# Jutho/Strided.jl

Hardware: AMD Instinct MI355X
Metric: GB/s effective HBM for @strided permutedims!+broadcast, 32^4 fp64 (higher is better)
Workload: dtype f64

## Files before the change

### strided.jl_amd/csrc/smr_api.cpp

```cpp
#include <algorithm>
#include <cstdio>
#include <cstring>
#include <atomic>
#include <list>
#include <memory>
#include <mutex>
#include <string>
#include <unordered_map>
#include <vector>

#include "smr_dispatch.h"
#include "smr_group.h"

namespace smr {

static thread_local std::string g_last_error;

int set_error(int code, const std::string& msg) {
    g_last_error = msg;
    return code;
}
int hip_error(hipError_t e, const char* what) {
    g_last_error = std::string(what) + ": " + hipGetErrorString(e);
    return e == hipErrorOutOfMemory ? SMR_ENOMEM : (e == hipErrorNoDevice ? SMR_ENODEVICE : SMR_EHIP);
// ... 316 lines not shown
        const uint32_t align = (uint32_t)((uintptr_t)p->ops[k].base & 255u);
        int32_t acls = k;
        const char* ak = (const char*)p->ops[k].base + p->ops[k].offset * (int64_t)dtype_size(p->ops[k].dtype);
        for (int j = 0; j < k; ++j)
            if ((const char*)p->ops[j].base + p->ops[j].offset * (int64_t)dtype_size(p->ops[j].dtype) == ak) {
                acls = j;
                break;
            }
        put(&acls, sizeof acls);
        put(&cls, sizeof cls);
        put(&align, sizeof align);
        put(&p->ops[k].offset, sizeof(int64_t));
        put(p->ops[k].strides, sizeof(int64_t) * (size_t)p->N);
        put(&p->ops[k].dtype, sizeof(int32_t));
        put(&p->ops[k].conj, sizeof(int32_t));
    }
    put(&p->fprog_len, sizeof(int32_t));
    if (p->fprog && p->fprog_len > 0) put(p->fprog, (size_t)(2 * p->fprog_len));
    put(&p->nconsts, sizeof(int32_t));
    if (p->fconsts && p->nconsts > 0) put(p->fconsts, sizeof(double) * (size_t)(2 * p->nconsts));
    put(&p->redop, sizeof(int32_t));
    put(&p->initop, sizeof(int32_t));
    put(p->initarg, sizeof p->initarg);
    put(&p->stream, sizeof(void*));
    return s;
}

void cache_clear_locked(Cache& c, std::vector<PlanRef>& dropped) {
    for (auto& kv : c.lru) dropped.push_back(std::move(kv.second));
    c.lru.clear();
    c.map.clear();
}

struct OptionField {
    const char* name;
    i64 Options::*field;
};
const OptionField OPTION_FIELDS[] = {
    {"force_family", &Options::force_family},
    {"jit", &Options::jit},
    {"max_lds_bytes", &Options::max_lds_bytes},
    {"tile_log2", &Options::tile_log2},
    {"tile_order", &Options::tile_order},
    {"tile_block", &Options::tile_block},
    {"tile_block_xcd", &Options::tile_block_xcd},
    {"tiled_vec", &Options::tiled_vec},
    {"tiled_uavec", &Options::tiled_uavec},
    {"tiled_edge_first", &Options::tiled_edge_first},
    {"tiled_persist", &Options::tiled_persist},
    {"tiled_persist_wpc", &Options::tiled_persist_wpc},
    {"tiled_persist_min", &Options::tiled_persist_min},
    {"tiled_xpose", &Options::tiled_xpose},
    {"tiled_gorder", &Options::tiled_gorder},
    {"orbit", &Options::orbit},
    {"orbit_lg", &Options::orbit_lg},
    {"orbit_min", &Options::orbit_min},
    {"orbit_few", &Options::orbit_few},
    {"orbit_minrun", &Options::orbit_minrun},
    {"orbit_group", &Options::orbit_group},
    {"orbit_pipe", &Options::orbit_pipe},
    {"orbit_wgs", &Options::orbit_wgs},
    {"orbit_pair", &Options::orbit_pair},
    {"orbit_pack", &Options::orbit_pack},
    {"flat", &Options::flat},
    {"flat_wide", &Options::flat_wide},
    {"flat2", &Options::flat2},
    {"flat2_pair", &Options::flat2_pair},
    {"flat2_bytes", &Options::flat2_bytes},
    {"flat2_lead_bytes", &Options::flat2_lead_bytes},
    {"flat2_long", &Options::flat2_long},
    {"flatb", &Options::flatb},
    {"stream_ua", &Options::stream_ua},
    {"stream_pack_rows", &Options::stream_pack_rows},
    {"nt_store", &Options::nt_store},
    {"nt_stream_min", &Options::nt_stream_min},
    {"reduce_blocks", &Options::reduce_blocks},
    {"reduce_part_wgs", &Options::reduce_part_wgs},
    {"reduce_part_kind", &Options::reduce_part_kind},
    {"reduce_single", &Options::reduce_single},
    {"reduce_row_floor", &Options::reduce_row_floor},
    {"reduce_row_dense", &Options::reduce_row_dense},
    {"reduce_col_txlog", &Options::reduce_col_txlog},
    {"reduce_col_exact", &Options::reduce_col_exact},
    {"reduce_col_narrow", &Options::reduce_col_narrow},
    {"nt_load", &Options::nt_load},
    {"eager_direct", &Options::eager_direct},
    {"eager_self_release", &Options::eager_self_release},
    {"seq_self_release", &Options::seq_self_release},
    {"self_release_max_bytes", &Options::self_release_max_bytes},
    {"self_release_max_total", &Options::self_release_max_total},
    {"allreduce_f64", &Options::allreduce_f64},
};

i64 Options::*option_field(const std::string& n) {
    for (const OptionField& f : OPTION_FIELDS)
        if (n == f.name) return f.field;
    return nullptr;
}

int tile_lg_dim(const std::string& n) {
    return n.size() == 8 && n.rfind("tile_lg", 0) == 0 && n[7] >= '0' && n[7] <= '7' ? n[7] - '0' : -1;
}
}

extern "C" {

// ... 443 lines not shown
```

### strided.jl_amd/csrc/smr_internal.h

```cpp
#pragma once

#ifndef SMR_JIT
#include <hip/hip_runtime.h>

#include <array>
#include <memory>
#include <mutex>
#include <string>
#include <vector>

#include "../../include/strided_hip.h"
#else
#include "strided_hip.h"
#endif

#include <cstdint>

namespace smr {

typedef int64_t i64;
constexpr int MAXN = SMR_MAXN;
constexpr int MAXM = SMR_MAXM;
constexpr int MAXIN = SMR_MAXM - 1;
constexpr int STACK = 8;
constexpr int MAXG = 4;
constexpr int FLATB_MAXP = 512;
constexpr int TILED_NG = 4;

#ifndef SMR_JIT
int set_error(int code, const std::string& msg);
int hip_error(hipError_t e, const char* what);
#endif

inline int dtype_size(int dt) {
    switch (dt) {
        case SMR_F32: return 4;
        case SMR_F64: return 8;
        case SMR_C32: return 8;
        case SMR_C64: return 16;
        case SMR_I8: case SMR_U8: case SMR_BOOL: return 1;
        case SMR_I16: case SMR_U16: return 2;
        case SMR_I32: case SMR_U32: return 4;
        case SMR_I64: case SMR_U64: return 8;
    }
    return 0;
}

struct ProgD {
    int32_t len;
    int32_t nconst;
    uint8_t code[2 * SMR_MAXPROG];
    double consts[2 * SMR_MAXCONST];
};

struct JitConsts {
    double c[2 * SMR_MAXCONST];
};

enum FKind : int {
    FK_PROG = 0,
    FK_IDENT = 1,
    FK_ADD2 = 2,
    FK_ADD3 = 3,
    FK_ADD4 = 4,
    FK_SCALE = 5,
    FK_SYM = 6,
    FK_AXPY = 7,
    FK_AXPBY = 8,
    FK_ABS2 = 9,
    FK_MUL2 = 10,
    FK_EXPR5 = 11,
    FK_COUNT
};

enum Family : int {
    FAM_AUTO = 0,
    FAM_GENERIC = 1,
    FAM_STREAM = 2,
    FAM_TILED = 3,
    FAM_REDUCE_ALL = 4,
// ... 84 lines not shown
};

struct Flat2Plan {
    bool on = false;
    int kt = 1;
    bool shared = false;
    int R[2] = {1, 1}, TP[2] = {1, 1}, p[2] = {-1, -1};
    bool ingroup[2][MAXN] = {{false, false, false, false, false, false, false, false}, {false, false, false, false, false, false, false, false}};
    int32_t roff[2][64];
};

struct FlatBPlan {
    bool on = false;
    int g = 0, P = 0, K = 1;
    uint16_t srcoff[FLATB_MAXP];
};

struct StreamPlan {
    int vec = 1;
    bool vec_ua = false;
};

struct ReducePlan {
    int nparts = 1;
    size_t scratch_bytes = 0;
    int tr = 1;
    int kind = 0;
    int g0log = 0, g1log = 0;
    int txlog = 0;
    int col_tx = 0, col_v = 1;
    int col_y0 = 1, col_y1 = 1;
    int xsplit = 1, qsplit = 1;
};

struct Plan {
    Canon c;
    int family = FAM_GENERIC;
    FlatBPlan flatb;
    TilePlan tile;
    OrbitPlan orbit;
    FlatPlan flat;
    Flat2Plan flat2;
    StreamPlan stream;
    ReducePlan red;
    mutable bool eager_seen = false;
    void* scratch = nullptr;
    size_t counter_off = 0;
    struct FormCache {
        std::vector<unsigned char> args;
        void* tab = nullptr;
    };
    mutable std::shared_ptr<std::mutex> build_mu = std::make_shared<std::mutex>();
    mutable FormCache tiled_cache[4];
    mutable void* tiled_order = nullptr;
    mutable FormCache orbit_cache[2];
    mutable void* orbit_list = nullptr;
    mutable FormCache pair_cache;
    std::array<void**, 9> dev_tables() const {
        return {&tiled_cache[0].tab, &tiled_cache[1].tab, &tiled_cache[2].tab, &tiled_cache[3].tab, &tiled_order,
                &orbit_cache[0].tab, &orbit_cache[1].tab, &orbit_list, &pair_cache.tab};
    }
    struct ArgBlock {
        int launch = 0;
        std::vector<unsigned char> bytes;
        void* dev = nullptr;
        int dev_index = 0;
        unsigned long long epoch = 0;
    };
    mutable std::vector<ArgBlock> eager_args;
    std::string desc;
};

constexpr int RED_COUNTERS = 16384;
struct Options {
    i64 force_family = 0;
    i64 tile_log2 = 0;
    i64 tile_order = 1;
    i64 tile_block = -1;
    i64 tile_block_xcd = -1;
    i64 jit = 1;
    i64 reduce_col_txlog = 5;
    i64 reduce_part_wgs = 1024;
    i64 reduce_row_floor = -1;
    i64 flat_wide = 1;
    i64 flat2 = 1;
    i64 flat2_pair = 1;
    i64 flat2_bytes = 384;
    i64 flat2_lead_bytes = 512;
    i64 reduce_row_dense = 1;
    i64 reduce_col_exact = 1;
    i64 reduce_col_narrow = 1;
    i64 reduce_part_kind = -1;
    i64 reduce_single = 4;
    i64 reduce_blocks = 2048;
    i64 tiled_persist = 1;
    i64 tiled_persist_wpc = 0;
    i64 tiled_persist_min = 32;
    i64 eager_direct = 1;
    i64 flat2_long = 80;
    i64 flatb = 1;
    i64 stream_pack_rows = 1;
    i64 tiled_vec = 1;
    i64 tiled_edge_first = 1;
    i64 tiled_uavec = 1;
    i64 orbit = 1;
    i64 stream_ua = 1;
    i64 tiled_xpose = 1;
    i64 tiled_gorder = -1;
    i64 allreduce_f64 = 0;
    i64 eager_self_release = 1;
    i64 seq_self_release = 1;
    i64 self_release_max_total = (i64)128 << 20;
    i64 self_release_max_bytes = (i64)64 << 20;
    i64 orbit_lg = -1;
    i64 orbit_min = 150;
    i64 orbit_pipe = -1;
    i64 orbit_group = 2;
    i64 stamp_base = 0, stamp_cap = 0, stamp_used = 0;
    i64 flat = 1;
    i64 orbit_minrun = 16;
    i64 orbit_wgs = 0;
    i64 orbit_pair = 1;
    i64 orbit_pack = 1;
    i64 orbit_few = 40;
    i64 nt_store = -1;
    i64 nt_stream_min = 0;
    i64 nt_load = -1;
    i64 max_lds_bytes = 65536;
    i64 tile_lg[MAXN] = {-1, -1, -1, -1, -1, -1, -1, -1};
};
Options& options();

unsigned long long* stamp_next(size_t waves);

int canonicalise(const smr_problem* p, Canon& c);
int make_plan(const smr_problem* p, Plan& plan);
void describe(Plan& plan);

enum RedFold { RED_FOLD_EPILOGUE = 0, RED_FOLD_IN_LAUNCH = 1, RED_FOLD_SECOND_LAUNCH = 2 };
struct RedLaunch {
    int vec = 1;
    int fold = RED_FOLD_EPILOGUE;
    int nparts = 1;
    i64 groups = 0;
    int ctx = 0, cty = 0, cy0 = 0, cy1 = 0;
};
RedLaunch reduce_launch(const Plan& plan, void* const* bases, bool have_scratch);

struct TiledVariant {
    int V = 1;
    bool ua = false;
    int mode = 0;
    bool wide = false;
    int thrlog = 8;
    unsigned pgrid = 0;
};
TiledVariant tiled_variant(const Plan& plan, void* const* bases, int esize, bool mixed);

constexpr int SMR_JIT_UNAVAILABLE = 1000;
struct JitLaunch {
    const char* family;
    const char* tname;
    std::string entry;
    const char* argtype;
    unsigned grid = 1, block = 256;
    size_t lds = 0;
    const void* args = nullptr;
    size_t argsize = 0;
};
int jit_launch(const Canon& c, const JitLaunch& l, hipStream_t s);
int jit_compile_only(const Canon& c, const JitLaunch& l, size_t* code_size);
std::string jit_functor_source(const Canon& c, const char* tname);
bool jit_dry_run();
void jit_set_prepare(bool on);
bool jit_no_launch();
void jit_set_dry_run(bool on);
size_t jit_dry_code_size();
struct JitStats {
    long compiles = 0, hits = 0, failures = 0;
    double compile_ms = 0;
};
JitStats jit_stats();

int fence_for_foreign_work(hipStream_t s);

struct RecLaunch {
    const void* hostfn = nullptr;
    std::string kname;
    std::shared_ptr<void> keep;
    unsigned grid = 0, block = 0, lds = 0;
    int slice_kind = 0;
    unsigned slice_off = 0, slice_row = 0;
    bool self_released = false;
    std::vector<unsigned char> args;
};
std::vector<RecLaunch>* recorder();
struct Plan;
int eager_submit(const Plan& plan, std::vector<RecLaunch>& launches, const std::vector<std::pair<uintptr_t, uintptr_t>>& rd,
                 const std::vector<std::pair<uintptr_t, uintptr_t>>& wr, hipStream_t s);
long comm_stat(int which);
void count_launch();
int eager_fence_all();
void eager_note_hip_work(hipStream_t s);
void eager_forget_stream(hipStream_t s);
void eager_request_sys_acquire(hipStream_t s);
long eager_stat(int which);
bool eager_available(hipStream_t s);
int eager_fence_if_active();
bool eager_recent_writes_fit(uintptr_t dest_lo, uintptr_t dest_hi);
void mark_sliceable(int kind, unsigned off, unsigned row);
void mark_self_released();
void take_slice_mark(RecLaunch& r);
void set_recorder(std::vector<RecLaunch>* r, bool allow_self_release = false, bool eager = false);
bool want_self_release(const Plan& plan);

int upload_table(void** dst, const void* src, size_t bytes, const char* what);
int cu_count();

int launch_generic_map(const Plan& plan, void* const* bases, hipStream_t s);
int launch_stream_map(const Plan& plan, void* const* bases, hipStream_t s);
int launch_tiled_map(const Plan& plan, void* const* bases, hipStream_t s);
int launch_reduce_all(const Plan& plan, void* const* bases, hipStream_t s);
int launch_reduce_part(const Plan& plan, void* const* bases, hipStream_t s);
int launch_orbit_map(const Plan& plan, void* const* bases, hipStream_t s);
int launch_flat_map(const Plan& plan, void* const* bases, hipStream_t s);

#endif

}
```

### strided.jl_amd/csrc/smr_k_tiled.hip

```cpp
#ifndef SMR_JIT
#include <cstdio>
#include <cstdlib>
#include <vector>
#endif

#include "smr_dispatch.h"

#ifndef SMR_CT
#error "compile with -DSMR_CT=0..3 or 7"
#endif
#ifndef SMR_TILED_BITS
#define SMR_TILED_BITS 0
#endif
#ifndef SMR_TILED_NTL
#define SMR_TILED_NTL 0
#endif

namespace smr {

constexpr int MAXT = 5;
constexpr int NG = TILED_NG;
constexpr int EPL = 4;
constexpr int NORD16 = 512;

// ... 1118 lines not shown
    constexpr int T0 = 128, TQ = 32;
    if constexpr (is_jit<F>::value || !tr<T>::arith || sizeof(T) < 8 || (F::NIN >= 0 && F::NIN != 1)) {
        return SMR_EUNSUPPORTED;
    } else {
        if (!options().tiled_xpose) return SMR_EUNSUPPORTED;
        if (c.M != 2 || c.mixed || c.N < 3 || c.N > MAXN || t.nt != 2 || t.tilelog != 12 || t.staged[1] < 0 || !t.ord.empty()) return SMR_EUNSUPPORTED;
        if (t.tdim[0] != 0 || t.tlog[0] != 7 || t.tlog[1] != 5) return SMR_EUNSUPPORTED;
        const int q = t.tdim[1];
        if (c.strides[0][0] != 1 || c.strides[1][q] != 1 || c.dims[0] % T0 || c.dims[q] % TQ) return SMR_EUNSUPPORTED;
        if (tab.conj[0] || tab.conj[1]) return SMR_EUNSUPPORTED;
        if (c.algbytes < ((i64)512 << 20)) return SMR_EUNSUPPORTED;
        const i64 es = (i64)sizeof(T);
        if ((((uintptr_t)tab.base[0]) | ((uintptr_t)tab.base[1])) % 16) return SMR_EUNSUPPORTED;
        for (int d = 0; d < c.N; ++d) {
            if (d != 0 && (c.strides[0][d] * es) % 16) return SMR_EUNSUPPORTED;
            if (d != q && (c.strides[1][d] * es) % 16) return SMR_EUNSUPPORTED;
        }
        XposeArgs a;
        std::memset(&a, 0, sizeof a);
        a.src = (const char*)tab.base[1];
        a.dst = (char*)tab.base[0];
        a.src_row = c.strides[1][0] * es;
        a.dst_row = c.strides[0][q] * es;
        i64 grid = 1;
        int ng = 0;
        for (int i = 0; i < c.N; ++i) {
            const int d = t.gorder[i] >= 0 && t.gorder[i] < c.N ? t.gorder[i] : -1;
            if (d < 0) return SMR_EUNSUPPORTED;
            const i64 tile = d == 0 ? T0 : (d == q ? TQ : 1);
            const i64 n = c.dims[d] / tile;
            if (n <= 1) continue;
            if (n > 0xffffffffLL) return SMR_EUNSUPPORTED;
            a.ext[ng] = (uint32_t)n;
            a.sstep[ng] = c.strides[1][d] * es * tile;
            a.dstep[ng] = c.strides[0][d] * es * tile;
            grid *= n;
            ++ng;
        }
        {
            bool seen[MAXN] = {false};
            for (int i = 0; i < c.N; ++i) {
                if (seen[t.gorder[i]]) return SMR_EUNSUPPORTED;
                seen[t.gorder[i]] = true;
            }
        }
        a.ng = ng;
        if (grid < 1 || grid > 0x7fffffffLL) return SMR_EUNSUPPORTED;
        const size_t lds = (size_t)T0 * (TQ + 2) * sizeof(T);
        auto kern = k_xpose_big<T, F, V, T0, TQ>;
        return launch_native((const void*)kern, lds, "k_xpose_big", [&] { SMR_LAUNCH(kern, dim3((unsigned)grid), dim3(1024), lds, s, a, f); });
    }
}

template <class T, class F, bool MIXED>
static int go(const Plan& plan, void* const* bases, hipStream_t s, F f) {
    const Canon& c = plan.c;
    const TilePlan& t = plan.tile;
    const OpTab tab = make_optab(c, bases);
    if constexpr (!MIXED) {
        const int rc = try_xpose_big<T, F>(plan, s, f, tab);
        if (rc != SMR_EUNSUPPORTED) return rc;
    }
    if (t.tilelog != 10 && t.tilelog != 12) return set_error(SMR_EINVAL, "tiled: the planner must pick 1024- or 4096-element tiles");
    const TiledVariant tv = tiled_variant(plan, bases, (int)sizeof(T), MIXED);
    if (tv.thrlog == 8) return go_tl<T, F, MIXED, 8>(plan, s, f, tab, tv);
    return go_tl<T, F, MIXED, 10>(plan, s, f, tab, tv);
}

template <>
int launch_tiled_map_ct<SMR_CT>(const Plan& plan, void* const* bases, hipStream_t s) {
    typedef ct_type<SMR_CT>::type T;
    const Canon& c = plan.c;
    if (c.bitcopy) return with_bitcopy<SMR_CT>(c, [&](auto f) { return go<typename ident_elem<decltype(f)>::type, decltype(f), false>(plan, bases, s, f); });
    if (c.mixed) return with_prog<T>(c, [&](auto f) { return go<T, decltype(f), true>(plan, bases, s, f); });
    switch (c.fkind) {
        case FK_IDENT: return go<T, FIdent<T>, false>(plan, bases, s, FIdent<T>{});
        case FK_ADD2: return go<T, FAdd2<T>, false>(plan, bases, s, FAdd2<T>{});
        case FK_ADD3: return go<T, FAdd3<T>, false>(plan, bases, s, FAdd3<T>{});
        case FK_ADD4: return go<T, FAdd4<T>, false>(plan, bases, s, FAdd4<T>{});
        case FK_SCALE: return go<T, FScale<T>, false>(plan, bases, s, FScale<T>{hostmk<T>(c.fc[0], c.fc[1])});
        case FK_SYM: return go<T, FSym<T>, false>(plan, bases, s, FSym<T>{hostmk<T>(c.fc[0], c.fc[1])});
        case FK_AXPY: return go<T, FAxpy<T>, false>(plan, bases, s, FAxpy<T>{hostmk<T>(c.fc[0], c.fc[1])});
        case FK_AXPBY:
            return go<T, FAxpby<T>, false>(plan, bases, s, FAxpby<T>{hostmk<T>(c.fc[0], c.fc[1]), hostmk<T>(c.fc[2], c.fc[3])});
        default: break;
    }
    return with_prog<T>(c, [&](auto f) { return go<T, decltype(f), false>(plan, bases, s, f); });
}
#endif

}
```

### strided.jl_amd/csrc/smr_kmeta.cpp

```cpp
#include "smr_kmeta.h"

#include <algorithm>
#include <cstring>
#include <iterator>
#include <vector>

namespace smr {
namespace {

struct Cur {
    const unsigned char* p;
    const unsigned char* end;
    bool bad = false;

    bool need(size_t n) {
        if ((size_t)(end - p) < n) bad = true;
        return !bad;
    }
    uint64_t be(int n) {
        if (!need((size_t)n)) return 0;
        uint64_t v = 0;
        for (int i = 0; i < n; ++i) v = (v << 8) | p[i];
        p += n;
        return v;
// ... 64 lines not shown
                case 0xd9: str((size_t)be(1)); break;
                case 0xda: str((size_t)be(2)); break;
                case 0xdb: str((size_t)be(4)); break;
                case 0xdc: t.kind = ARR; t.i = (int64_t)be(2); break;
                case 0xdd: t.kind = ARR; t.i = (int64_t)be(4); break;
                case 0xde: t.kind = MAP; t.i = (int64_t)be(2); break;
                case 0xdf: t.kind = MAP; t.i = (int64_t)be(4); break;
                default: bad = true; break;
            }
        if (bad) t.kind = BAD;
        return t;
    }
    void skip_value() {
        uint64_t pending = 1;
        while (pending && !bad) {
            const Tok t = next();
            --pending;
            if (t.kind == ARR) pending += (uint64_t)t.i;
            else if (t.kind == MAP) pending += 2 * (uint64_t)t.i;
            else if (t.kind == BAD) bad = true;
        }
    }
};

bool is(const Cur::Tok& t, const char* s) { return t.kind == Cur::STR && t.n == std::strlen(s) && std::memcmp(t.s, s, t.n) == 0; }

void parse_arg(Cur& c, KernargLayout& L) {
    const Cur::Tok m = c.next();
    if (m.kind != Cur::MAP) {
        c.bad = true;
        return;
    }
    int64_t off = -1, size = 0;
    std::string kind;
    for (int64_t i = 0; i < m.i && !c.bad; ++i) {
        const Cur::Tok k = c.next();
        if (is(k, ".offset")) {
            const Cur::Tok v = c.next();
            if (v.kind == Cur::INT) off = v.i; else c.bad = true;
        } else if (is(k, ".size")) {
            const Cur::Tok v = c.next();
            if (v.kind == Cur::INT) size = v.i; else c.bad = true;
        } else if (is(k, ".value_kind")) {
            const Cur::Tok v = c.next();
            if (v.kind == Cur::STR) kind.assign(v.s, v.n); else c.bad = true;
        } else {
            c.skip_value();
        }
    }
    if (c.bad || off < 0) return;
    const int32_t o = (int32_t)off;
    if (kind.compare(0, 7, "hidden_") != 0) {
        L.explicit_end = std::max<int32_t>(L.explicit_end, (int32_t)(off + size));
        ++L.nargs_explicit;
        return;
    }
    static const char* const xyz[3] = {"_x", "_y", "_z"};
    for (int d = 0; d < 3; ++d) {
        if (kind == std::string("hidden_block_count") + xyz[d]) { L.block_count[d] = o; return; }
        if (kind == std::string("hidden_group_size") + xyz[d]) { L.group_size[d] = o; return; }
        if (kind == std::string("hidden_remainder") + xyz[d]) { L.remainder[d] = o; return; }
        if (kind == std::string("hidden_global_offset") + xyz[d]) { L.global_offset[d] = o; return; }
    }
    if (kind == "hidden_grid_dims") { L.grid_dims = o; return; }
    if (kind == "hidden_dynamic_lds_size") { L.dynamic_lds = o; return; }
    if (kind == "hidden_none" || kind == "hidden_private_base" || kind == "hidden_shared_base") return;
    L.needs_runtime = 1;
}

void parse_kernel(Cur& c, std::map<std::string, KernargLayout>& out) {
    const Cur::Tok m = c.next();
    if (m.kind != Cur::MAP) {
        c.bad = true;
        return;
    }
    KernargLayout L;
    std::string symbol, name;
    for (int64_t i = 0; i < m.i && !c.bad; ++i) {
        const Cur::Tok k = c.next();
        auto int_into = [&](int32_t& dst) {
            const Cur::Tok v = c.next();
            if (v.kind == Cur::INT) dst = (int32_t)v.i; else c.bad = true;
        };
        if (is(k, ".symbol")) {
            const Cur::Tok v = c.next();
            if (v.kind == Cur::STR) symbol.assign(v.s, v.n); else c.bad = true;
        } else if (is(k, ".name")) {
            const Cur::Tok v = c.next();
            if (v.kind == Cur::STR) name.assign(v.s, v.n); else c.bad = true;
        } else if (is(k, ".kernarg_segment_size")) {
            int_into(L.kernarg_size);
        } else if (is(k, ".private_segment_fixed_size")) {
            int_into(L.private_size);
        } else if (is(k, ".group_segment_fixed_size")) {
            int_into(L.group_static);
        } else if (is(k, ".args")) {
            const Cur::Tok a = c.next();
            if (a.kind != Cur::ARR) {
                c.bad = true;
                break;
            }
            for (int64_t j = 0; j < a.i && !c.bad; ++j) parse_arg(c, L);
        } else {
            c.skip_value();
        }
    }
// ... 188 lines not shown
```

### strided.jl_amd/csrc/smr_kmeta.h

```cpp
#pragma once

#include <cstddef>
#include <cstdint>
#include <map>
#include <string>

namespace smr {

struct KernargLayout {
    int32_t kernarg_size = 0;
    int32_t explicit_end = 0;
    int32_t nargs_explicit = 0;
    int32_t block_count[3] = {-1, -1, -1};
    int32_t group_size[3] = {-1, -1, -1};
    int32_t remainder[3] = {-1, -1, -1};
    int32_t global_offset[3] = {-1, -1, -1};
    int32_t grid_dims = -1;
    int32_t dynamic_lds = -1;
    int32_t needs_runtime = 0;
    int32_t private_size = 0, group_static = 0;
};

bool kmeta_parse(const void* elf, size_t bytes, std::map<std::string, KernargLayout>& out, std::string& why);

void kmeta_fill_hidden(const KernargLayout& layout, unsigned char* block, uint32_t grid, uint32_t block_size, uint32_t dyn_lds);

KernargLayout kmeta_v5_default(size_t explicit_end, size_t kernarg_size);

}
```

### strided.jl_amd/csrc/smr_plan.cpp

```cpp
#include <algorithm>
#include <array>
#include <cstdio>
#include <cstdlib>
#include <vector>

#include "smr_internal.h"

namespace smr {

constexpr i64 FLAT_GROUP_MAX = 64;

static int elem_bytes(const Canon& c) { return c.bitcopy ? c.esize[0] : dtype_size(c.ct); }

static int ceil_log2(i64 v) {
    int l = 0;
    while (((i64)1 << l) < v) ++l;
    return l;
}

static i64 even_cut(i64 want, i64 n) {
    if (n <= 1 || want <= 1) return 1;
    if (n <= 2 * want) return n;
    const i64 per = (n + want - 1) / want;
    return (n + per - 1) / per;
// ... 1385 lines not shown
    TiledVariant v;
    v.thrlog = t.tilelog - 2;
    for (int k = 0; k < c.M && !v.wide; ++k) {
        long double span = 0;
        for (int j = 0; j < t.nt; ++j) {
            const i64 st = c.strides[k][t.tdim[j]];
            if (st < 0) v.wide = true;
            span += (long double)st * (((i64)1 << t.tlog[j]) - 1) * c.esize[k];
        }
        if (span >= 4294967296.0L) v.wide = true;
    }
    if (!v.wide && !mixed && esize < 16 && o.tiled_vec) {
        const int V = 16 / esize > 4 ? 4 : 16 / esize;
        int vlog = 0;
        while ((1 << vlog) < V) ++vlog;
        bool whole = V > 1, ua = V > 1 && o.tiled_uavec && esize >= 4;
        for (int k = 0; k < c.M && (whole || ua); ++k) {
            const bool staged = k > 0 && t.staged[k] >= 0;
            const int j0 = staged ? t.order[k][0] : 0;
            const int d0 = t.tdim[j0];
            const uintptr_t base = (uintptr_t)(bases ? bases[c.orig[k]] : c.base[k]) + (uintptr_t)(c.offsets[k] * (i64)c.esize[k]);
            if (t.tlog[j0] < vlog || c.strides[k][d0] != 1) whole = ua = false;
            if (c.dims[d0] % V || base % ((size_t)V * esize)) whole = false;
            for (int d = 0; d < c.N && whole; ++d)
                if (d != d0 && (c.strides[k][d] % V)) whole = false;
            if (c.dims[d0] < V || base % esize) ua = false;
        }
        if (whole || ua) {
            v.V = V;
            v.ua = !whole;
        }
    }
    bool ragged = false;
    for (int j = 0; j < t.nt; ++j)
        if (c.dims[t.tdim[j]] & (((i64)1 << t.tlog[j]) - 1)) ragged = true;
    bool pv = false;
    if (v.V > 1)
        for (int k = 0; k < c.M; ++k) {
            const int j0 = (k > 0 && t.staged[k] >= 0) ? t.order[k][0] : 0;
            if (c.dims[t.tdim[j0]] % v.V) pv = true;
        }
    if (ragged) v.mode = !t.ord.empty() ? 7 : (pv ? 9 : 1);
    else v.mode = t.ord.empty() ? 0 : 2;
    if (!t.origins32) v.mode = 7;
    if ((v.mode & 1) == 0 && o.tiled_persist && !t.no_persist && !v.ua) {
        const size_t lds = (size_t)t.nstaged * ((size_t)1 << t.tilelog) * esize;
        const i64 grid = t.ord.empty() ? t.grid : (i64)t.ord.size();
        i64 wpc = std::min<i64>(2048 >> v.thrlog, lds ? (i64)(160 * 1024 / lds) : 8);
        wpc = std::max<i64>(1, std::min<i64>(wpc, 4));
        if (o.tiled_persist_wpc > 0) wpc = o.tiled_persist_wpc;
        const i64 cap = (i64)cu_count() * wpc / 8 * 8;
        if ((i64)(unsigned)grid >= cap * o.tiled_persist_min && cap >= 8) v.pgrid = (unsigned)cap;
    }
    return v;
}

void describe(Plan& plan) {
    const Canon& c = plan.c;
    static const char* fam[] = {"auto", "generic", "stream", "tiled", "reduce_all", "reduce_part", "orbit", "flat"};
    static const char* fk[] = {"prog", "ident", "add2", "add3", "add4", "scale", "sym", "axpy", "axpby", "abs2", "mul2", "expr5"};
    static const char* ct[] = {"f32", "f64", "c32", "c64"};
    char buf[1024];
    int n = std::snprintf(buf, sizeof buf, "family=%s ct=%s%s f=%s N=%d M=%d dims=", fam[plan.family], c.ct == SMR_I64 ? "i64" : ct[c.ct & 3],
                          c.bitcopy ? "(bitcopy)" : (c.mixed ? "(mixed)" : ""), fk[c.fkind], c.N, c.M);
    for (int i = 0; i < c.N; ++i) n += std::snprintf(buf + n, sizeof buf - n, "%s%lld", i ? "x" : "", (long long)c.dims[i]);
    if (plan.family == FAM_TILED) {
        n += std::snprintf(buf + n, sizeof buf - n, " tile=");
        for (int j = 0; j < plan.tile.nt; ++j)
            n += std::snprintf(buf + n, sizeof buf - n, "%sd%d:%d", j ? "," : "", plan.tile.tdim[j], 1 << plan.tile.tlog[j]);
        n += std::snprintf(buf + n, sizeof buf - n, " staged=%d lds=%zu grid=%lld threads=%d", plan.tile.nstaged,
                           plan.tile.lds_bytes, (long long)plan.tile.grid, plan.tile.threads);
        if (!plan.tile.ord.empty()) n += std::snprintf(buf + n, sizeof buf - n, " order=orbits:%d", plan.tile.ord_groups);
        if (plan.tile.tilelog == 10 || plan.tile.tilelog == 12) {
            const TiledVariant v = tiled_variant(plan, nullptr, elem_bytes(c), c.mixed && !c.bitcopy);
            n += std::snprintf(buf + n, sizeof buf - n, " vec=%d%s mode=%d%s%s", v.V, v.ua ? "(element-aligned)" : "", v.mode, v.wide ? " wide" : "",
                               v.pgrid ? " pipe" : "");
        }
    } else if (plan.family == FAM_ORBIT) {
        const OrbitPlan& ob = plan.orbit;
        n += std::snprintf(buf + n, sizeof buf - n, " tile=");
        bool first = true;
        for (int d = 0; d < c.N; ++d)
            if (ob.lg[d] > 0) {
                n += std::snprintf(buf + n, sizeof buf - n, "%sd%d:%d", first ? "" : ",", d, 1 << ob.lg[d]);
                first = false;
            }
        n += std::snprintf(buf + n, sizeof buf - n, " group=%d orbits=%d lds=%zu grid=%zu", ob.ng, ob.norbits, ob.lds_bytes, ob.wmap.size());
        if (ob.pair_ok) n += std::snprintf(buf + n, sizeof buf - n, " pair_grid=%zu", ob.pmap.size() / 2);
    } else if (plan.family == FAM_FLAT && plan.flatb.on) {
        n += std::snprintf(buf + n, sizeof buf - n, " batched block=%d(d0..d%d) blocks_per_wg=%d", plan.flatb.P, plan.flatb.g - 1, plan.flatb.K);
    } else if (plan.family == FAM_FLAT && plan.flat2.on) {
        const Flat2Plan& f2 = plan.flat2;
        n += std::snprintf(buf + n, sizeof buf - n, " two-sided dest_run=%dx%d(d%d) input_run=%dx%d(d%d)%s", f2.R[0], f2.TP[0], f2.p[0], f2.R[1], f2.TP[1], f2.p[1],
                           f2.shared ? " shared-dim" : "");
    } else if (plan.family == FAM_FLAT) {
        const FlatPlan& fp = plan.flat;
        n += std::snprintf(buf + n, sizeof buf - n, " flat_side=%s run=%dx%d(d%d)%s line=d%d:%d", fp.dir == 0 ? "dest" : "input", fp.R, 1 << fp.tplog, fp.p,
                           fp.fuse ? "+line" : (fp.lshare ? " shared-lead" : ""), fp.q, 1 << fp.tqlog);
    } else if (plan.family == FAM_STREAM) {
        n += std::snprintf(buf + n, sizeof buf - n, " vec=%d%s", plan.stream.vec, plan.stream.vec_ua ? "(element-aligned+tail)" : "");
    } else if (plan.family == FAM_REDUCE_ALL) {
        n += std::snprintf(buf + n, sizeof buf - n, " blocks=%d", plan.red.nparts);
    } else if (plan.family == FAM_REDUCE_PART) {
        static const char* kinds[] = {"general", "row", "col"};
        n += std::snprintf(buf + n, sizeof buf - n, " nout=%lld form=%s lanes_per_out=%d split=%d", (long long)c.nout, kinds[plan.red.kind],
                           plan.red.tr, plan.red.nparts);
        if (plan.red.kind == 2 && plan.red.col_tx) n += std::snprintf(buf + n, sizeof buf - n, " lanes=%dx%d", plan.red.col_tx, 256 / plan.red.col_tx);
    }
    if (plan.family == FAM_REDUCE_ALL || plan.family == FAM_REDUCE_PART) {
        static const char* folds[] = {"epilogue", "in-launch", "second-launch"};
        const RedLaunch r = reduce_launch(plan, nullptr, true);
        n += std::snprintf(buf + n, sizeof buf - n, " vec=%d fold=%s", r.vec, folds[r.fold]);
    }
    if (c.int_wraps) n += std::snprintf(buf + n, sizeof buf - n, " int_wraps=%d", c.int_wraps);
    std::snprintf(buf + n, sizeof buf - n, " algbytes=%lld", (long long)c.algbytes);
    plan.desc = buf;
}

}
```

### strided.jl_amd/csrc/smr_seq.cpp

```cpp
#include <sched.h>

#include <algorithm>
#include <cstdio>
#include <cstdlib>
#include <cstring>

#include "smr_direct.h"

using namespace smr;

struct SeqItem {
    smr_plan* plan;
    smr_group* group;
    bool has_bases;
    void* bases[SMR_MAXM];
};
struct SeqPacket {
    hsa_kernel_dispatch_packet_t pk;
    bool barrier;
    bool acquire;
    bool self_released;
};
struct smr_seq {
    std::vector<SeqItem> items;
// ... 71 lines not shown
    k.self_release_max_total = options().self_release_max_total;
    return k;
}

int seq_record(smr_seq* q, std::vector<Rec>& recs, std::vector<SchedExec>& ex) {
    for (const SeqItem& it : q->items)
        if (int rc = seq_execute_item(it, nullptr, true)) return rc;
    ex = seq_footprints(q);
    const bool allow_self = schedule(ex, seq_knobs(q)).cache_resident;
    for (size_t i = 0; i < q->items.size(); ++i) {
        set_recorder(&recs[i].launches, allow_self);
        int rc = seq_execute_item(q->items[i], nullptr, false);
        set_recorder(nullptr);
        if (rc) return rc;
        if (recs[i].launches.empty()) return set_error(SMR_EINVAL, "smr_seq: an item recorded no launch");
        const RecLaunch& l0 = recs[i].launches[0];
        ex[i].nlaunch = (int)recs[i].launches.size();
        ex[i].grid = l0.grid;
        ex[i].sliceable = l0.slice_kind != 0;
        ex[i].all_self = true;
        for (const RecLaunch& l : recs[i].launches) ex[i].all_self = ex[i].all_self && l.self_released;
    }
    return SMR_OK;
}

bool seq_resolve(smr_seq* q, Direct& d, std::vector<Rec>& recs) {
    for (Rec& r : recs)
        for (const RecLaunch& l : r.launches) {
            if (l.keep) q->keep.push_back(l.keep);
            KernelRef k;
            if (!resolve_launch(d, l, k, &q->why_not_aql)) return false;
            r.refs.push_back(k);
        }
    return true;
}

int seq_kernargs(smr_seq* q, std::vector<Rec>& recs, const Schedule& sc) {
    size_t total = 0;
    for (size_t i = 0; i < recs.size(); ++i)
        for (size_t j = 0; j < recs[i].launches.size(); ++j) {
            recs[i].offs.push_back(total);
            total += recs[i].blocksize(j) * (size_t)sc.nslices[i];
        }
    std::vector<unsigned char> host(total, 0);
    for (size_t i = 0; i < recs.size(); ++i)
        for (size_t j = 0; j < recs[i].launches.size(); ++j) {
            const RecLaunch& l = recs[i].launches[j];
            const int ns = sc.nslices[i];
            for (int s2 = 0; s2 < ns; ++s2) {
                unsigned lo = 0, hi = l.grid;
                if (ns > 1) slice_range(l.grid, ns, s2, lo, hi);
                unsigned char* b = host.data() + recs[i].offs[j] + (size_t)s2 * recs[i].blocksize(j);
                fill_kernarg_image(recs[i].refs[j], l, hi - lo, b, recs[i].blocksize(j));
                if (ns > 1 && l.slice_kind == 1) {
                    uint32_t v;
                    std::memcpy(&v, b + l.slice_off, 4);
                    v += lo;
                    std::memcpy(b + l.slice_off, &v, 4);
                } else if (ns > 1 && l.slice_kind == 2) {
                    uint64_t v;
                    std::memcpy(&v, b + l.slice_off, 8);
                    v += (uint64_t)lo * l.slice_row;
                    std::memcpy(b + l.slice_off, &v, 8);
                }
#if SMR_STAMP
                if (ns > 1 && l.args.size() >= 8) {
                    uint64_t sp = 0;
                    std::memcpy(&sp, b + l.args.size() - 8, 8);
                    if (sp) {
                        sp += (uint64_t)lo * ((l.block + 63) / 64) * 16;
                        std::memcpy(b + l.args.size() - 8, &sp, 8);
                    }
                }
#endif
            }
        }
    if (q->d_kernargs) (void)hipFree(q->d_kernargs);
    q->d_kernargs = nullptr;
    hipError_t e = hipMalloc(&q->d_kernargs, total ? total : 256);
    if (e != hipSuccess) return hip_error(e, "hipMalloc(sequence kernargs)");
    e = hipMemcpy(q->d_kernargs, host.data(), total, hipMemcpyHostToDevice);
    if (e != hipSuccess) return hip_error(e, "hipMemcpy(sequence kernargs)");
    return SMR_OK;
}

int seq_first_acquire_scope(const std::vector<SchedExec>& ex, int device) {
    for (const SchedExec& r : ex)
        for (const auto& x : r.rd) {
            hipPointerAttribute_t at;
            std::memset(&at, 0, sizeof at);
            const bool local = x.second > x.first && hipPointerGetAttributes(&at, (const void*)x.first) == hipSuccess && at.type == hipMemoryTypeDevice &&
                               !at.isManaged && at.device == device;
            if (!local) {
                (void)hipGetLastError();
                return HSA_FENCE_SCOPE_SYSTEM;
            }
        }
    return HSA_FENCE_SCOPE_AGENT;
}

int seq_build(smr_seq* q) {
    for (auto& v : q->packets) v.clear();
    q->keep.clear();
    q->aql = false;
    q->n_any = q->n_barrier = q->n_acquire = q->n_self_released = 0;
    q->nq = 0;
    q->nsliced = 0;
    q->device = current_device();
    Direct& d = direct_of(q->device);
    if (!d.ok) {
        std::lock_guard<std::mutex> g(d.why_mu);
// ... 395 lines not shown
```

Baseline: 7836.

## Add lean specialized tiled transpose kernel for identity copies with swizzled LDS

Adds a specialized 'lean' tiled kernel for plain two-operand identity/bitcopy permutations with 1024-element tiles and power-of-two tile grids. It uses 16-byte vector loads and stores, a compact packed geometry argument, an XOR swizzle chosen on the host to reduce LDS bank conflicts, and shift/mask block-index decoding instead of the general tiled kernel's machinery. The aim is to cut per-thread address arithmetic and register pressure in the transpose path. It also adds kernarg offset tracking so sliced sequence launches can patch the new block-offset argument, which adds complexity and narrow eligibility checks.

```diff
diff --git a/strided.jl_amd/csrc/smr_api.cpp b/strided.jl_amd/csrc/smr_api.cpp
--- a/strided.jl_amd/csrc/smr_api.cpp
+++ b/strided.jl_amd/csrc/smr_api.cpp
@@ -392,6 +392,7 @@
     {"tiled_persist_min", &Options::tiled_persist_min},
     {"tiled_xpose", &Options::tiled_xpose},
     {"tiled_gorder", &Options::tiled_gorder},
+    {"tiled_lean", &Options::tiled_lean},
     {"orbit", &Options::orbit},
     {"orbit_lg", &Options::orbit_lg},
     {"orbit_min", &Options::orbit_min},
diff --git a/strided.jl_amd/csrc/smr_internal.h b/strided.jl_amd/csrc/smr_internal.h
--- a/strided.jl_amd/csrc/smr_internal.h
+++ b/strided.jl_amd/csrc/smr_internal.h
@@ -26,6 +26,7 @@
 constexpr int MAXG = 4;
 constexpr int FLATB_MAXP = 512;
 constexpr int TILED_NG = 4;
+constexpr int TILED_LEAN_NG = 3;
 
 #ifndef SMR_JIT
 int set_error(int code, const std::string& msg);
@@ -216,6 +217,7 @@
     };
     mutable std::shared_ptr<std::mutex> build_mu = std::make_shared<std::mutex>();
     mutable FormCache tiled_cache[4];
+    mutable FormCache lean_cache;
     mutable void* tiled_order = nullptr;
     mutable FormCache orbit_cache[2];
     mutable void* orbit_list = nullptr;
@@ -270,6 +272,7 @@
     i64 orbit = 1;
     i64 stream_ua = 1;
     i64 tiled_xpose = 1;
+    i64 tiled_lean = 1;
     i64 tiled_gorder = -1;
     i64 allreduce_f64 = 0;
     i64 eager_self_release = 1;
@@ -318,6 +321,7 @@
     bool wide = false;
     int thrlog = 8;
     unsigned pgrid = 0;
+    bool lean = false;
 };
 TiledVariant tiled_variant(const Plan& plan, void* const* bases, int esize, bool mixed);
 
@@ -388,6 +392,8 @@
 int launch_reduce_part(const Plan& plan, void* const* bases, hipStream_t s);
 int launch_orbit_map(const Plan& plan, void* const* bases, hipStream_t s);
 int launch_flat_map(const Plan& plan, void* const* bases, hipStream_t s);
+struct OpTab;
+int launch_tiled_lean(const Plan& plan, const OpTab& tab, int esize, bool conj, hipStream_t s);
 
 #endif
 
diff --git a/strided.jl_amd/csrc/smr_k_lean.hip b/strided.jl_amd/csrc/smr_k_lean.hip
--- /dev/null
+++ b/strided.jl_amd/csrc/smr_k_lean.hip
@@ -0,0 +1,234 @@
+#include <cstdio>
+#include <cstdlib>
+#include <cstring>
+#include <vector>
+
+#include "smr_dispatch.h"
+
+namespace smr {
+
+struct LeanArgs {
+    const char* src;
+    char* dst;
+    uint32_t blk0;
+    uint32_t geo;
+    uint32_t sa, db;
+    uint32_t step[6];
+};
+constexpr int LEAN_BLK0_ARG = 2;
+constexpr int LEAN_NG = TILED_LEAN_NG;
+
+typedef uint32_t lean_u4 __attribute__((ext_vector_type(4)));
+
+template <int ES, int SMODE>
+__global__ void __launch_bounds__(256) k_tiled_lean(const char* src, char* dst, uint32_t blk0, uint32_t geo, uint32_t sa, uint32_t db, uint32_t ss0,
+                                                    uint32_t ds0, uint32_t ss1, uint32_t ds1, uint32_t ss2, uint32_t ds2 SMR_STAMP_PARAM) {
+    SMR_STAMP_BEGIN
+    constexpr int V = 16 / ES;
+    constexpr int VLOG = V == 4 ? 2 : (V == 2 ? 1 : 0);
+    constexpr int ELOG = ES == 4 ? 2 : (ES == 8 ? 3 : 4);
+    constexpr int NREP = 4 / V;
+    constexpr int EW = ES / 4;
+    constexpr uint32_t FMASK = (uint32_t)(128 / ES - 1) & ~(uint32_t)(V - 1);
+    extern __shared__ __attribute__((aligned(16))) unsigned char smem_lean[];
+    const uint32_t tid = threadIdx.x;
+    const uint32_t la = geo & 15u, lb = 10u - la;
+    const uint32_t fs1 = (geo >> 24) & 15u, fd = (geo >> 28) & 7u;
+    const uint32_t fs2 = fd == 7u ? 31u : fs1 + 1u + fd;
+    const uint32_t cmask = geo & 0x80000000u;
+
+    uint32_t b = blockIdx.x + blk0;
+    uint64_t so = 0, dof = 0;
+    {
+        const uint32_t sst[LEAN_NG] = {ss0, ss1, ss2}, dst_[LEAN_NG] = {ds0, ds1, ds2};
+#pragma unroll
+        for (int g = 0; g < LEAN_NG; ++g) {
+            const uint32_t lg = (geo >> (4 + 5 * g)) & 31u;
+            const uint32_t tc = b & ((1u << lg) - 1u);
+            b >>= lg;
+            so += (uint64_t)tc * sst[g];
+            dof += (uint64_t)tc * dst_[g];
+        }
+    }
+    const char* sp = src + so;
+    char* dp = dst + dof;
+
+    lean_u4 x[NREP];
+#pragma unroll
+    for (int r = 0; r < NREP; ++r) {
+        const uint32_t e = ((uint32_t)(r << 8) | tid) << VLOG;
+        const uint32_t ib = e & ((1u << lb) - 1u), ia = e >> lb;
+        x[r] = *reinterpret_cast<const lean_u4*>(sp + (ia * sa + (ib << ELOG)));
+    }
+    struct alignas(ES) Elem {
+        uint32_t w[EW];
+    };
+    Elem* lds = reinterpret_cast<Elem*>(smem_lean);
+#pragma unroll
+    for (int r = 0; r < NREP; ++r) {
+        const uint32_t e = ((uint32_t)(r << 8) | tid) << VLOG;
+        const uint32_t ib = e & ((1u << lb) - 1u), ia = e >> lb;
+#pragma unroll
+        for (int h = 0; h < V; ++h) {
+            const uint32_t l = ia + ((ib + (uint32_t)h) << la);
+            Elem v;
+#pragma unroll
+            for (int w = 0; w < EW; ++w) v.w[w] = x[r][h * EW + w];
+            if constexpr (ES >= 8) v.w[EW - 1] ^= cmask;
+            lds[l ^ (((l >> fs1) ^ (l >> fs2)) & FMASK)] = v;
+        }
+    }
+    __syncthreads();
+#pragma unroll
+    for (int r = 0; r < NREP; ++r) {
+        const uint32_t e = ((uint32_t)(r << 8) | tid) << VLOG;
+        const uint32_t ia = e & ((1u << la) - 1u), ib = e >> la;
+        const uint32_t l = e ^ (((e >> fs1) ^ (e >> fs2)) & FMASK);
+        x[r] = *reinterpret_cast<const lean_u4*>(smem_lean + ((size_t)l << ELOG));
+        char* p = dp + (ib * db + (ia << ELOG));
+        if constexpr (SMODE == 2)
+            store_vec_wt<lean_u4>(p, x[r]);
+        else
+            store_vec_ct<SMODE == 1, lean_u4>(p, x[r]);
+    }
+    if constexpr (SMODE == 2) self_release_wait();
+    SMR_STAMP_END
+}
+
+static int lean_rank(const uint32_t* v, int n) {
+    uint32_t basis[32];
+    int r = 0;
+    for (int i = 0; i < n; ++i) {
+        uint32_t x = v[i];
+        for (int j = 0; j < r; ++j)
+            if ((x ^ basis[j]) < x) x ^= basis[j];
+        if (x) {
+            basis[r++] = x;
+            for (int j = r - 1; j > 0 && basis[j] > basis[j - 1]; --j) std::swap(basis[j], basis[j - 1]);
+        }
+    }
+    return r;
+}
+
+static void lean_fold(int esize, int la, int lb, uint32_t& fs1_out, uint32_t& fd_out, int* cost_out) {
+    int w = 0, vlog = 0;
+    while ((esize << w) < 128) ++w;
+    while ((esize << vlog) < 16) ++vlog;
+    const uint32_t fmask = ((1u << w) - 1u) & ~((1u << vlog) - 1u);
+    int inbit[10];
+    for (int i = 0; i < lb; ++i) inbit[i] = la + i;
+    for (int i = 0; i < la; ++i) inbit[lb + i] = i;
+    auto image = [&](int bit, int s1, int s2) {
+        uint32_t v = 1u << bit;
+        if (bit >= s1) v ^= (1u << (bit - s1)) & fmask;
+        if (s2 < 31 && bit >= s2) v ^= (1u << (bit - s2)) & fmask;
+        return v;
+    };
+    int best = 1 << 30;
+    fs1_out = (uint32_t)w;
+    fd_out = 7;
+    for (int s1 = w; s1 < 10; ++s1)
+        for (int d = 0; d <= 7; ++d) {
+            const int s2 = d == 7 ? 31 : s1 + 1 + d;
+            if (d < 7 && s2 >= 10) continue;
+            uint32_t img[8];
+            int cost = 0;
+            for (int i = 0; i < w; ++i) img[i] = image(inbit[vlog + i], s1, s2) & ((1u << w) - 1u);
+            cost += (1 << (w - lean_rank(img, w))) - 1;
+            for (int i = 0; i < 4; ++i) img[i] = image(vlog + i, s1, s2) & ((1u << (w + 1)) - 1u);
+            cost += (1 << (4 - lean_rank(img, 4))) - 1;
+            if (cost < best) {
+                best = cost;
+                fs1_out = (uint32_t)s1;
+                fd_out = (uint32_t)d;
+            }
+        }
+    if (cost_out) *cost_out = best;
+}
+
+static int build_lean_args(const Plan& plan, const OpTab& tab, int esize, bool conj, LeanArgs& a, unsigned& grid) {
+    const Canon& c = plan.c;
+    const TilePlan& t = plan.tile;
+    grid = (unsigned)t.grid;
+    Plan::FormCache& cached = plan.lean_cache;
+    if (cached.args.size() == sizeof a) {
+        std::memcpy(&a, cached.args.data(), sizeof a);
+        a.src = (const char*)tab.base[1];
+        a.dst = (char*)tab.base[0];
+        return SMR_OK;
+    }
+    std::memset(&a, 0, sizeof a);
+    if (t.nt != 2 || t.tilelog != 10 || c.M != 2) return set_error(SMR_EINVAL, "tiled: the lean form was picked for a plan it does not cover");
+    const int la = t.tlog[0], lb = t.tlog[1], q = t.tdim[1];
+    const i64 es = esize;
+    a.src = (const char*)tab.base[1];
+    a.dst = (char*)tab.base[0];
+    a.sa = (uint32_t)(c.strides[1][0] * es);
+    a.db = (uint32_t)(c.strides[0][q] * es);
+    uint32_t fs1 = 0, fd = 7;
+    int cost = 0;
+    lean_fold(esize, la, lb, fs1, fd, &cost);
+    if (std::getenv("SMR_DEBUG_SWIZZLE")) std::fprintf(stderr, "[smr] tiled lean swizzle: fs1=%u fd=%u conflict cost=%d\n", fs1, fd, cost);
+    uint32_t geo = (uint32_t)la | (fs1 << 24) | (fd << 28) | (conj ? 0x80000000u : 0u);
+    int ng = 0;
+    bool seen[MAXN] = {false};
+    auto add = [&](int d) -> int {
+        if (d < 0 || d >= c.N || seen[d] || t.ntiles[d] <= 1) return SMR_OK;
+        seen[d] = true;
+        int lg = 0;
+        while (((i64)1 << lg) < t.ntiles[d]) ++lg;
+        if (ng >= LEAN_NG || ((i64)1 << lg) != t.ntiles[d]) return set_error(SMR_EINVAL, "tiled: the lean form was picked for a grid it does not cover");
+        const i64 tile = d == 0 ? (i64)1 << la : (d == q ? (i64)1 << lb : 1);
+        geo |= (uint32_t)lg << (4 + 5 * ng);
+        a.step[2 * ng] = (uint32_t)(c.strides[1][d] * tile * es);
+        a.step[2 * ng + 1] = (uint32_t)(c.strides[0][d] * tile * es);
+        ++ng;
+        return SMR_OK;
+    };
+    for (int i = 0; i < c.N; ++i)
+        if (int rc = add(t.gorder[i])) return rc;
+    for (int d = 0; d < c.N; ++d)
+        if (int rc = add(d)) return rc;
+    a.geo = geo;
+    if (!jit_dry_run()) {
+        cached.args.resize(sizeof a);
+        std::memcpy(cached.args.data(), &a, sizeof a);
+    }
+    return SMR_OK;
+}
+
+template <int ES, int SMODE>
+static void lean_launch(const LeanArgs& a, unsigned grid, hipStream_t s) {
+    auto kern = k_tiled_lean<ES, SMODE>;
+    const size_t lds = (size_t)1024 * ES;
+    SMR_LAUNCH(kern, dim3(grid), dim3(256), lds, s, a.src, a.dst, a.blk0, a.geo, a.sa, a.db, a.step[0], a.step[1], a.step[2], a.step[3], a.step[4], a.step[5] SMR_STAMP_ARG(grid, 256));
+}
+
+template <int ES>
+static void lean_launch_es(const LeanArgs& a, unsigned grid, int nts, hipStream_t s) {
+    if (nts == 2) lean_launch<ES, 2>(a, grid, s);
+    else if (nts) lean_launch<ES, 1>(a, grid, s);
+    else lean_launch<ES, 0>(a, grid, s);
+}
+
+int launch_tiled_lean(const Plan& plan, const OpTab& tab, int esize, bool conj, hipStream_t s) {
+    if (esize != 4 && esize != 8 && esize != 16) return set_error(SMR_EINVAL, "tiled: no lean kernel for this element size");
+    LeanArgs a;
+    unsigned grid = 0;
+    if (int rc = build_lean_args(plan, tab, esize, conj, a, grid)) return rc;
+    const Canon& c = plan.c;
+    const Options& o = options();
+    int nts = (o.nt_store > 0) ? 1 : 0;
+    if (o.nt_store < 0) nts = (((i64)1 << plan.tile.tlog[0]) * esize >= 128) ? 1 : 0;
+    if (o.nt_store == 2 || want_self_release(plan)) nts = 2;
+    (void)c;
+    return launch_native(nullptr, 0, "k_tiled_lean", [&] {
+        mark_sliceable(3, (unsigned)LEAN_BLK0_ARG, (unsigned)offsetof(LeanArgs, blk0));
+        if (nts == 2) mark_self_released();
+        if (esize == 4) lean_launch_es<4>(a, grid, nts, s);
+        else if (esize == 8) lean_launch_es<8>(a, grid, nts, s);
+        else lean_launch_es<16>(a, grid, nts, s);
+    });
+}
+
+}
diff --git a/strided.jl_amd/csrc/smr_k_tiled.hip b/strided.jl_amd/csrc/smr_k_tiled.hip
--- a/strided.jl_amd/csrc/smr_k_tiled.hip
+++ b/strided.jl_amd/csrc/smr_k_tiled.hip
@@ -1194,6 +1194,9 @@
     }
 }
 
+template <class F> struct is_ident_functor { static constexpr bool value = false; };
+template <class E> struct is_ident_functor<FIdent<E>> { static constexpr bool value = true; };
+
 template <class T, class F, bool MIXED>
 static int go(const Plan& plan, void* const* bases, hipStream_t s, F f) {
     const Canon& c = plan.c;
@@ -1205,6 +1208,9 @@
     }
     if (t.tilelog != 10 && t.tilelog != 12) return set_error(SMR_EINVAL, "tiled: the planner must pick 1024- or 4096-element tiles");
     const TiledVariant tv = tiled_variant(plan, bases, (int)sizeof(T), MIXED);
+    if constexpr (!MIXED && is_ident_functor<F>::value) {
+        if (tv.lean) return launch_tiled_lean(plan, tab, (int)sizeof(T), tr<T>::cx && (tab.conj[0] != 0) != (tab.conj[1] != 0), s);
+    }
     if (tv.thrlog == 8) return go_tl<T, F, MIXED, 8>(plan, s, f, tab, tv);
     return go_tl<T, F, MIXED, 10>(plan, s, f, tab, tv);
 }
diff --git a/strided.jl_amd/csrc/smr_kmeta.cpp b/strided.jl_amd/csrc/smr_kmeta.cpp
--- a/strided.jl_amd/csrc/smr_kmeta.cpp
+++ b/strided.jl_amd/csrc/smr_kmeta.cpp
@@ -140,6 +140,7 @@
     const int32_t o = (int32_t)off;
     if (kind.compare(0, 7, "hidden_") != 0) {
         L.explicit_end = std::max<int32_t>(L.explicit_end, (int32_t)(off + size));
+        if (L.nargs_explicit < KernargLayout::MAX_ARG_OFF) L.arg_off[L.nargs_explicit] = o;
         ++L.nargs_explicit;
         return;
     }
diff --git a/strided.jl_amd/csrc/smr_kmeta.h b/strided.jl_amd/csrc/smr_kmeta.h
--- a/strided.jl_amd/csrc/smr_kmeta.h
+++ b/strided.jl_amd/csrc/smr_kmeta.h
@@ -11,6 +11,8 @@
     int32_t kernarg_size = 0;
     int32_t explicit_end = 0;
     int32_t nargs_explicit = 0;
+    static constexpr int MAX_ARG_OFF = 24;
+    int32_t arg_off[MAX_ARG_OFF] = {-1, -1, -1, -1, -1, -1, -1, -1, -1, -1, -1, -1, -1, -1, -1, -1, -1, -1, -1, -1, -1, -1, -1, -1};
     int32_t block_count[3] = {-1, -1, -1};
     int32_t group_size[3] = {-1, -1, -1};
     int32_t remainder[3] = {-1, -1, -1};
diff --git a/strided.jl_amd/csrc/smr_plan.cpp b/strided.jl_amd/csrc/smr_plan.cpp
--- a/strided.jl_amd/csrc/smr_plan.cpp
+++ b/strided.jl_amd/csrc/smr_plan.cpp
@@ -1461,6 +1461,28 @@
         const i64 cap = (i64)cu_count() * wpc / 8 * 8;
         if ((i64)(unsigned)grid >= cap * o.tiled_persist_min && cap >= 8) v.pgrid = (unsigned)cap;
     }
+    if (o.tiled_lean && c.M == 2 && !mixed && (c.fkind == FK_IDENT || c.bitcopy) && (esize == 4 || esize == 8 || esize == 16) &&
+        v.mode == 0 && !v.wide && !v.pgrid && v.thrlog == 8 && t.origins32 && t.ord.empty() && t.nt == 2 && t.staged[1] >= 0 && t.tdim[0] == 0 &&
+        t.order[1][0] == 1 && v.V == (esize == 16 ? 1 : 16 / esize) && !v.ua) {
+        const int q = t.tdim[1], vlog = esize == 16 ? 0 : (esize == 8 ? 1 : 2);
+        bool ok = c.strides[0][0] == 1 && c.strides[1][q] == 1 && t.tlog[0] >= vlog && t.tlog[1] >= vlog && t.tlog[0] + t.tlog[1] == 10;
+        int ng = 0;
+        for (int d = 0; d < c.N && ok; ++d) {
+            if (t.ntiles[d] > 1) ++ng;
+            if (t.ntiles[d] & (t.ntiles[d] - 1)) ok = false;
+            for (int k = 0; k < 2; ++k) {
+                const i64 sb = c.strides[k][d] * (i64)esize;
+                if (sb < 0 || sb >= ((i64)1 << 32)) ok = false;
+                if (d != (k == 0 ? 0 : q) && (sb & 15)) ok = false;
+            }
+        }
+        for (int k = 0; k < 2 && ok; ++k) {
+            const uintptr_t base = (uintptr_t)(bases ? bases[c.orig[k]] : c.base[k]) + (uintptr_t)(c.offsets[k] * (i64)c.esize[k]);
+            if (base & 15) ok = false;
+        }
+        if ((c.conj[0] || c.conj[1]) && (c.bitcopy || !(c.ct == SMR_C32 || c.ct == SMR_C64))) ok = false;
+        v.lean = ok && ng <= TILED_LEAN_NG;
+    }
     return v;
 }
 
@@ -1482,8 +1504,8 @@
         if (!plan.tile.ord.empty()) n += std::snprintf(buf + n, sizeof buf - n, " order=orbits:%d", plan.tile.ord_groups);
         if (plan.tile.tilelog == 10 || plan.tile.tilelog == 12) {
             const TiledVariant v = tiled_variant(plan, nullptr, elem_bytes(c), c.mixed && !c.bitcopy);
-            n += std::snprintf(buf + n, sizeof buf - n, " vec=%d%s mode=%d%s%s", v.V, v.ua ? "(element-aligned)" : "", v.mode, v.wide ? " wide" : "",
-                               v.pgrid ? " pipe" : "");
+            n += std::snprintf(buf + n, sizeof buf - n, " vec=%d%s mode=%d%s%s%s", v.V, v.ua ? "(element-aligned)" : "", v.mode, v.wide ? " wide" : "",
+                               v.pgrid ? " pipe" : "", v.lean ? " lean" : "");
         }
     } else if (plan.family == FAM_ORBIT) {
         const OrbitPlan& ob = plan.orbit;
diff --git a/strided.jl_amd/csrc/smr_seq.cpp b/strided.jl_amd/csrc/smr_seq.cpp
--- a/strided.jl_amd/csrc/smr_seq.cpp
+++ b/strided.jl_amd/csrc/smr_seq.cpp
@@ -147,11 +147,18 @@
                 if (ns > 1) slice_range(l.grid, ns, s2, lo, hi);
                 unsigned char* b = host.data() + recs[i].offs[j] + (size_t)s2 * recs[i].blocksize(j);
                 fill_kernarg_image(recs[i].refs[j], l, hi - lo, b, recs[i].blocksize(j));
-                if (ns > 1 && l.slice_kind == 1) {
+                if (ns > 1 && (l.slice_kind == 1 || l.slice_kind == 3)) {
+                    unsigned off = l.slice_off;
+                    if (l.slice_kind == 3) {
+                        const KernargLayout& lay = recs[i].refs[j].layout;
+                        off = l.slice_row;
+                        if (l.slice_off < (unsigned)KernargLayout::MAX_ARG_OFF && lay.arg_off[l.slice_off] >= 0) off = (unsigned)lay.arg_off[l.slice_off];
+                    }
+                    if ((size_t)off + 4 > l.args.size()) return set_error(SMR_EINVAL, "smr_seq: the block-offset argument of a sliced launch lies outside its arguments");
                     uint32_t v;
-                    std::memcpy(&v, b + l.slice_off, 4);
+                    std::memcpy(&v, b + off, 4);
                     v += lo;
-                    std::memcpy(b + l.slice_off, &v, 4);
+                    std::memcpy(b + off, &v, 4);
                 } else if (ns > 1 && l.slice_kind == 2) {
                     uint64_t v;
                     std::memcpy(&v, b + l.slice_off, 8);
```

After: 8290 (median of 4 runs). 5.8% higher.
